# ronen-halevy/yolo-v3-tf2

Hardware: AMD Instinct MI355X
Metric: images/sec at 416x416 batch=64, f32 (full YOLOv3 detect: conv stack + decode + NMS) (higher is better)
Workload: dtype f32

## Files before the change

### include/y3.h

```cpp
#ifndef Y3_H
#define Y3_H

#include <stddef.h>
#include <stdint.h>

#ifdef __cplusplus
extern "C" {
#endif

typedef int y3_status;
enum {
    Y3_OK = 0,
    Y3_ERR_INVALID = -1,
    Y3_ERR_HIP = -2,
    Y3_ERR_OOM = -3,
    Y3_ERR_STATE = -4,
    Y3_ERR_NODEVICE = -5,
    Y3_ERR_COMM = -6,
    Y3_ERR_INTERNAL = -7
};

enum { Y3_DTYPE_F32 = 0, Y3_DTYPE_BF16 = 1, Y3_DTYPE_F32X3 = 2, Y3_DTYPE_F32X2 = 3, Y3_DTYPE_F16 = 4, Y3_DTYPE_I8 = 5 };

int y3_version(void);
// ... 37 lines not shown
                        const y3_conv_desc *convs, int n_convs, const y3_aux_desc *aux, int n_aux,
                        int input_tensor, const int32_t outputs[3], int nclasses, y3_net **out);
void y3_net_destroy(y3_net *net);

y3_status y3_net_set_conv_weights(y3_net *net, int conv_slot, const float *w, const float *gamma,
                                  const float *beta, const float *mean, const float *var, const float *bias,
                                  float eps);

y3_status y3_net_set_tile(y3_net *net, int conv_slot, int tile);
y3_status y3_net_set_tile_bf16(y3_net *net, int conv_slot, int tile);
y3_status y3_net_set_tile_x3(y3_net *net, int conv_slot, int tile);
y3_status y3_net_set_tile_x2(y3_net *net, int conv_slot, int tile);
y3_status y3_net_set_lanes(y3_net *net, int lanes);
y3_status y3_net_set_xcd_mode(y3_net *net, int mode);
y3_status y3_net_set_k_chunk(y3_net *net, int channels);
y3_status y3_net_set_low_latency(y3_net *net, int on);
y3_status y3_net_set_split_k(y3_net *net, int conv_slot, int S);
int y3_net_get_split_k(const y3_net *net, int conv_slot);
int y3_choose_split_k(long long tiles, int k_tiles, int n_cus, long long slab_bytes_per_slice);
y3_status y3_net_set_low_latency_bf16(y3_net *net, int on);
y3_status y3_net_set_split_k_bf16(y3_net *net, int conv_slot, int S);
int y3_net_get_split_k_bf16(const y3_net *net, int conv_slot);
y3_status y3_net_set_low_latency_f16(y3_net *net, int on);
y3_status y3_net_set_split_k_f16(y3_net *net, int conv_slot, int S);
int y3_net_get_split_k_f16(const y3_net *net, int conv_slot);
y3_status y3_net_keep_activations(y3_net *net, int keep);
y3_status y3_net_set_stem_fusion(y3_net *net, int on);
y3_status y3_net_set_stem_fusion_f16(y3_net *net, int on);
y3_status y3_net_measure_sclk(y3_net *net, const float *images_dev, int batch, float *const grids_dev[3], int forwards,
                              float *mhz_out, void *stream);
// ... 107 lines not shown
```

### yolo-v3-tf2_amd/_lib.py

```python
from __future__ import annotations

import ctypes as C
import os

from . import PACKAGE_DIR

LIB_PATH = os.environ.get("Y3_LIB_PATH") or os.path.join(PACKAGE_DIR, "lib", "liby3hip.so")

Y3_OK = 0
Y3_DTYPE_F32, Y3_DTYPE_BF16, Y3_DTYPE_F32X3, Y3_DTYPE_F32X2, Y3_DTYPE_F16, Y3_DTYPE_I8 = 0, 1, 2, 3, 4, 5
DTYPE_TAGS = {Y3_DTYPE_F32: "f32", Y3_DTYPE_BF16: "bf16", Y3_DTYPE_F32X3: "f32x3", Y3_DTYPE_F32X2: "f32x2", Y3_DTYPE_F16: "f16", Y3_DTYPE_I8: "i8"}
TILES_I8_BUILT = (8, 10, 11, 12, 17, 19, 24, 26, 27, 29)
TILES_X2_BUILT = (0, 1, 2, 3, 4, 8, 12, 26, 27)
TILES_X3_BUILT = (0, 1, 2, 3, 4, 8, 9, 12, 13, 14)
Y3_AUX_ADD, Y3_AUX_UPSAMPLE2X, Y3_AUX_CONCAT = 0, 1, 2
_Z = (0, 0, 0, 0)
TILES = [_Z, _Z, _Z, _Z, _Z, _Z,
         (128, 128, 4, 1), _Z, (256, 32, 4, 1), (128, 64, 4, 1), (64, 128, 4, 1), (64, 64, 4, 1),
         (128, 128, 8, 1), _Z, _Z, _Z,
         _Z, (128, 64, 8, 1), _Z, _Z,
         _Z, _Z, _Z,
         (128, 128, 4, 1), _Z,
         _Z,
         (64, 128, 4, 2), (64, 64, 4, 2), _Z, _Z, _Z,
# ... 57 lines not shown
    "y3_device_count": (_i, []),
    "y3_tile_built": (_i, [_i, _i]),
    "y3_net_create": (_i, [C.POINTER(TensorDesc), _i, C.POINTER(C.c_int32), _i, C.POINTER(ConvDesc), _i,
                           C.POINTER(AuxDesc), _i, _i, C.POINTER(C.c_int32), _i, C.POINTER(_vp)]),
    "y3_net_destroy": (None, [_vp]),
    "y3_net_set_conv_weights": (_i, [_vp, _i, _fp, _fp, _fp, _fp, _fp, _fp, _f]),
    "y3_net_set_tile": (_i, [_vp, _i, _i]),
    "y3_net_set_tile_bf16": (_i, [_vp, _i, _i]),
    "y3_net_set_tile_x3": (_i, [_vp, _i, _i]),
    "y3_net_set_tile_x2": (_i, [_vp, _i, _i]),
    "y3_net_set_early_chunk": (_i, [_vp, _i, _i]),
    "y3_net_keep_activations": (_i, [_vp, _i]),
    "y3_net_set_lanes": (_i, [_vp, _i]),
    "y3_net_set_xcd_mode": (_i, [_vp, _i]),
    "y3_net_set_k_chunk": (_i, [_vp, _i]),
    "y3_net_set_stem_fusion": (_i, [_vp, _i]),
    "y3_net_set_low_latency": (_i, [_vp, _i]),
    "y3_net_set_split_k": (_i, [_vp, _i, _i]),
    "y3_net_get_split_k": (_i, [_vp, _i]),
    "y3_choose_split_k": (_i, [C.c_longlong, _i, _i, C.c_longlong]),
    "y3_net_set_low_latency_bf16": (_i, [_vp, _i]),
    "y3_net_set_split_k_bf16": (_i, [_vp, _i, _i]),
    "y3_net_get_split_k_bf16": (_i, [_vp, _i]),
    "y3_net_set_low_latency_f16": (_i, [_vp, _i]),
    "y3_net_set_split_k_f16": (_i, [_vp, _i, _i]),
    "y3_net_get_split_k_f16": (_i, [_vp, _i]),
    "y3_net_set_stem_fusion_f16": (_i, [_vp, _i]),
    "y3_net_measure_sclk": (_i, [_vp, _vp, _i, C.POINTER(_vp), _i, _fp, _vp]),
    "y3_net_measure_sclk_conv": (_i, [_vp, _vp, _i, C.POINTER(_vp), _i, _i, _fp, _vp]),
    "y3_net_measure_sclk_all": (_i, [_vp, _vp, _i, C.POINTER(_vp), _i, _fp, C.POINTER(C.c_double), C.POINTER(C.c_double), _vp]),
# ... 92 lines not shown
```

### yolo-v3-tf2_amd/csrc/conv_common.h

```cpp
#pragma once
#include "y3_device.h"
#include "y3_kernels.h"

namespace y3 {

struct TileOrigin { int b0, ho0, wo0; float rcpW, rcpH; };

__device__ __forceinline__ TileOrigin tile_origin(const ConvArgs &p, int m0)
{
    TileOrigin t;
    const int HoWo = p.Ho * p.Wo;
    t.b0 = m0 / HoWo;
    const int r0 = m0 - t.b0 * HoWo;
    t.ho0 = r0 / p.Wo;
    t.wo0 = r0 - t.ho0 * p.Wo;
    t.rcpW = 1.0f / (float)p.Wo;
    t.rcpH = 1.0f / (float)p.Ho;
    return t;
}

__device__ __forceinline__ void tile_row(const ConvArgs &p, const TileOrigin &t, int x, int &b, int &ho, int &wo)
{
    const int qx = (int)(((float)x + 0.5f) * t.rcpW);
    wo = x - qx * p.Wo;
// ... 9 lines not shown
    int b, ho, wo;
    tile_row(p, t, x, b, ho, wo);
    if (CONCAT) {
        const int H0 = p.up0 ? (p.H >> 1) : p.H, W0 = p.up0 ? (p.W >> 1) : p.W;
        const int h0 = p.up0 ? (ho >> 1) : ho, w0 = p.up0 ? (wo >> 1) : wo;
        aoff = ((b * H0 + h0) * W0 + w0) * EPC * p.C0;
        aoff1 = ((b * p.H + ho) * p.W + wo) * EPC * c1;
        ahw = (m < p.M) ? 0 : (int)0x80000000;
    } else {
        const int hi0 = ho * p.stride - p.pad, wi0 = wo * p.stride - p.pad;
        aoff = ((b * p.H + hi0) * p.W + wi0) * EPC * p.Cin;
        ahw = (m < p.M) ? ((hi0 << 16) | (wi0 & 0xffff)) : (int)0x80000000;
    }
}

template <int LPR>
__device__ __forceinline__ int swizzled_chunk(int row, int chunk)
{
    static_assert(LPR == 2 || LPR == 4 || LPR == 8, "16-byte chunks per LDS row");
    constexpr int SHIFT = (LPR == 8) ? 1 : (LPR == 4) ? 2 : 3;
    return chunk ^ ((row >> SHIFT) & (LPR - 1));
}

__device__ __forceinline__ constexpr int mfma32_row(int e, int fh = 0) { return 4 * fh + (e & 3) + 8 * (e >> 2); }
__device__ __forceinline__ constexpr int mfma16_row(int e, int fh, int mb = 0) { return 16 * mb + 4 * fh + e; }

}
```

### yolo-v3-tf2_amd/csrc/conv_f32.hip

```cpp
#include <algorithm>
#include <type_traits>

#include "conv_common.h"

namespace y3 {

static constexpr int BK = 32;
static constexpr int lds_row(int dma) { return dma ? BK : BK + 4; }

__device__ __forceinline__ f32x4 buf_load16(__amdgpu_buffer_rsrc_t r, unsigned voff, int soff)
{
    u32x4 v = __builtin_amdgcn_raw_buffer_load_b128(r, (int)voff, soff, 0);
    return __builtin_bit_cast(f32x4, v);
}

#ifdef Y3_PHASE_STAMPS
__device__ unsigned long long y3_dbg32_stamps[8 * 32768];
__device__ int y3_dbg32_sel_k = -1;
#define Y3_STAMP32(k) do { if (threadIdx.x == 0 && blockIdx.x < 32768 && p.K == y3_dbg32_sel_k) y3_dbg32_stamps[blockIdx.x * 8 + (k)] = __builtin_amdgcn_s_memrealtime(); } while (0)
#else
#define Y3_STAMP32(k) do { } while (0)
#endif

template <int TM, int TN, int WR, int WC, bool CONCAT, int STAGES, int MINW = 1, int DMA = 0, bool SPLIT = false>
__global__ __launch_bounds__(64 * WR * WC, MINW) void conv_f32_mfma(const ConvArgs p)
{
    static_assert(!SPLIT || (!DMA && STAGES == 1), "the split-K form is built for the register-staged single-stage tiles");
    Y3_STAMP32(0);
#ifdef Y3_PHASE_STAMPS
    if (threadIdx.x == 0 && blockIdx.x < 32768 && p.K == y3_dbg32_sel_k) {
        y3_dbg32_stamps[blockIdx.x * 8 + 5] = __builtin_amdgcn_s_getreg((31 << 11) | 4);
        y3_dbg32_stamps[blockIdx.x * 8 + 6] = __builtin_amdgcn_s_getreg((31 << 11) | 20);
    }
#endif
    static_assert(DMA || STAGES == 1, "register-staged operand loads are single-stage; two stages need the LDS-DMA loads");
    constexpr int LDS_ROW = lds_row(DMA);
    constexpr int BM = 32 * TM * WR;
    constexpr int BN = 32 * TN * WC;
    constexpr int NT = 64 * WR * WC;
    constexpr int RP = NT / 8;
    constexpr int AP = BM / RP;
    constexpr int BP = BN / RP;
    static_assert(BM % RP == 0 && BN % RP == 0 && AP >= 1 && BP >= 1, "tile too small for the thread count");
    constexpr int STAGE = (BM + BN) * LDS_ROW;
    extern __shared__ __attribute__((aligned(16))) float smem[];

    const int tid = threadIdx.x;
    if constexpr (!SPLIT) clk_stamp_entry(p.clk_stamps);
    const int lane = tid & 63;
    const int wave = __builtin_amdgcn_readfirstlane(tid >> 6);
    const int wr = wave / WC, wc = wave % WC;

    const int nwg = gridDim.x;
    const int bid = blockIdx.x, xcd = bid & 7;
    const int logical = xcd_contiguous_tile(bid, nwg);
    const int tilesN = p.CoutPad / BN;
    const int kt0 = SPLIT ? (int)blockIdx.y * (p.K / BK) / (int)gridDim.y : 0;
    const int KT = SPLIT ? ((int)blockIdx.y + 1) * (p.K / BK) / (int)gridDim.y - kt0 : p.K / BK;
    const __amdgpu_buffer_rsrc_t rs0 = buffer_rsrc(p.src0, p.src0_bytes);
    const __amdgpu_buffer_rsrc_t rs1 = buffer_rsrc(CONCAT ? p.src1 : p.src0, CONCAT ? p.src1_bytes : p.src0_bytes);
    const __amdgpu_buffer_rsrc_t rsw = buffer_rsrc(p.wpk, p.w_bytes);
    const unsigned OOB0 = p.src0_bytes, OOB1 = CONCAT ? p.src1_bytes : p.src0_bytes;

    const __amdgpu_buffer_rsrc_t rsd = buffer_rsrc(p.dst, p.dst_bytes);
    const __amdgpu_buffer_rsrc_t rsr = buffer_rsrc(p.residual ? p.residual : p.dst, p.dst_bytes);
    const int fr = lane & 31, fh = lane >> 5;

    int mt = logical / tilesN, nt = logical - mt * tilesN;
    if (p.xcd_gn > 0) {
        const int gn = p.xcd_gn, gm = 8 / gn;
        const int tilesM = (p.M + BM - 1) / BM;
        const int xm = xcd / gn, xn = xcd - xm * gn;
        const int nb = tilesN / gn;
        const int mlo = xm * tilesM / gm, mhi = (xm + 1) * tilesM / gm;
        const int j = bid >> 3;
        const int lm = j / nb;
        mt = mlo + lm;
        nt = xn * nb + (j - lm * nb);
        if (mt >= mhi) return;
    }
    const int m0 = mt * BM, n0 = nt * BN;

    const int lrow = tid >> 3;
    const int lchunk = DMA ? swizzled_chunk<8>(lrow, tid & 7) * 4 : (tid & 7) * 4;
    int aoff[AP];
    int aoff1[CONCAT ? AP : 1];
    int ahw[AP];
    const int C1 = p.Cin - p.C0;
    const TileOrigin org = tile_origin(p, m0);
#pragma unroll
    for (int i = 0; i < AP; ++i)
        gather_row<CONCAT, 1>(p, org, m0 + i * RP + lrow, org.wo0 + i * RP + lrow, C1, aoff[i], aoff1[CONCAT ? i : 0], ahw[i]);
    unsigned boff[BP];
#pragma unroll
    for (int j = 0; j < BP; ++j) boff[j] = (unsigned)((n0 + j * RP + lrow) * p.K + lchunk) * 4u;

    const int CK = (!CONCAT && p.k_chunk > 0 && p.k_chunk < p.Cin) ? p.k_chunk : p.Cin;
    int kglob = 0;
    int tap = 0;
    int c0 = 0;
    int cend = CK;
    const int taps = p.ksize * p.ksize;
    if constexpr (SPLIT) {
        const int tpc = CK / BK, per_chunk = taps * tpc;
        const int chunk = kt0 / per_chunk, r = kt0 - chunk * per_chunk;
        tap = r / tpc;
        c0 = chunk * CK + (r - tap * tpc) * BK;
        cend = (chunk + 1) * CK;
        kglob = tap * p.Cin + c0;
    }
    unsigned avoff[AP];
    unsigned okmask[CONCAT ? 1 : AP];
    unsigned abase4[CONCAT ? 1 : AP];
    unsigned avoff1[CONCAT ? AP : 1];
    auto set_tap = [&]() {
        if (CONCAT) {
#pragma unroll
            for (int i = 0; i < AP; ++i) {
                avoff[i] = (ahw[i] < 0) ? OOB0 : (unsigned)(aoff[i] + lchunk) * 4u;
                avoff1[i] = (ahw[i] < 0) ? OOB1 : (unsigned)(aoff1[i] + lchunk) * 4u;
            }
        } else {
            const int u = tap / p.ksize, v = tap - u * p.ksize;
            const unsigned toff4 = (unsigned)((u * p.W + v) * p.Cin) * 4u;
#pragma unroll
            for (int i = 0; i < AP; ++i) avoff[i] = ((okmask[i] >> tap) & 1u) ? abase4[i] + toff4 : OOB0;
        }
    };
    if (!CONCAT) {
#pragma unroll
        for (int i = 0; i < AP; ++i) {
            unsigned mk = 0;
            if (ahw[i] >= 0 || (ahw[i] >> 16) != -32768) {
                const int hi0 = ahw[i] >> 16, wi0 = (int)(short)(ahw[i] & 0xffff);
                if (p.ksize == 3) {
                    const unsigned H = (unsigned)p.H, W = (unsigned)p.W;
                    const unsigned rm = ((unsigned)hi0 < H ? 7u : 0u) | ((unsigned)(hi0 + 1) < H ? 56u : 0u) | ((unsigned)(hi0 + 2) < H ? 448u : 0u);
                    const unsigned cm = ((unsigned)wi0 < W ? 1u : 0u) | ((unsigned)(wi0 + 1) < W ? 2u : 0u) | ((unsigned)(wi0 + 2) < W ? 4u : 0u);
                    mk = rm & (cm * 73u);
                } else {
                    for (int u = 0; u < p.ksize; ++u)
                        for (int v = 0; v < p.ksize; ++v)
                            if ((unsigned)(hi0 + u) < (unsigned)p.H && (unsigned)(wi0 + v) < (unsigned)p.W) mk |= 1u << (u * p.ksize + v);
                }
            }
            okmask[i] = mk;
            abase4[i] = (unsigned)(aoff[i] + lchunk) * 4u;
        }
    }
    set_tap();

    auto advance_k = [&]() {
        c0 += BK;
        if (c0 == cend) {
            ++tap;
            if (!CONCAT && tap == taps && cend != p.Cin) {
                tap = 0;
                cend += CK;
            }
            c0 = cend - CK;
            if (!CONCAT) set_tap();
        }
        kglob = tap * p.Cin + c0;
    };

    f32x4 ra[AP], rb[BP];
    auto fetch_dma = [&](int buf) {
        float *sa = smem + buf * STAGE + wave * 8 * LDS_ROW;
        float *sb = sa + BM * LDS_ROW;
        if (CONCAT && c0 >= p.C0) {
#pragma unroll
            for (int i = 0; i < AP; ++i)
// ... 48 lines not shown
        asm volatile("s_waitcnt vmcnt(0)" ::: "memory");
    } else {
        fetch();
        stage(0);
    }
    __syncthreads();
    Y3_STAMP32(2);

    const int a_frag = (wr * 32 * TM + fr) * LDS_ROW + (DMA ? 0 : fh * 4);
    const int b_frag = BM * LDS_ROW + (wc * 32 * TN + fr) * LDS_ROW + (DMA ? 0 : fh * 4);
    int foff[4];
#pragma unroll
    for (int q = 0; q < 4; ++q) foff[q] = DMA ? swizzled_chunk<8>(fr, 2 * q + fh) * 4 : q * 8;

    const bool interior = (m0 + BM <= p.M) && (n0 + BN <= p.Cout);
    const int row_bytes = p.Cout * 4;

    for (int kt = 0; kt < KT; ++kt) {
        const int cur = (STAGES == 2) ? (kt & 1) : 0;
        if (DMA && STAGES == 2) {
            if (kt + 1 < KT) fetch_dma(cur ^ 1);
        } else if (!DMA) {
            if (kt + 1 < KT) fetch();
        }
        const float *sa = smem + cur * STAGE + a_frag;
        const float *sb = smem + cur * STAGE + b_frag;
#pragma unroll
        for (int q = 0; q < 4; ++q) {
            f32x4 fa[TM], fb[TN];
#pragma unroll
            for (int i = 0; i < TM; ++i) fa[i] = *reinterpret_cast<const f32x4 *>(sa + i * 32 * LDS_ROW + foff[q]);
// ... 41 lines not shown
                                                          mfma32_row(e) * slab_row_bytes, 0);
            }
        }
    } else {
    auto emit = [&](auto leaky_tag, auto res_tag, auto interior_tag) {
        constexpr bool LEAKY = decltype(leaky_tag)::value, RES = decltype(res_tag)::value;
        constexpr bool interior = decltype(interior_tag)::value;
#pragma unroll
        for (int j = 0; j < TN; ++j) {
            const int n = n0 + (wc * TN + j) * 32 + fr;
            const float sh = p.shift[n];
            const bool n_ok = n < p.Cout;
#pragma unroll
            for (int i = 0; i < TM; ++i) {
                const int mbase = m0 + (wr * TM + i) * 32 + 4 * fh;
                const unsigned vbase = (unsigned)(mbase * p.Cout + n) * 4u;
                unsigned off[16];
                if (!interior) {
#pragma unroll
                    for (int e = 0; e < 16; ++e) {
                        const int m = mbase + mfma32_row(e);
                        off[e] = (n_ok && m < p.M) ? (unsigned)(m * p.Cout + n) * 4u : p.dst_bytes;
                    }
                }
                float r[16];
                if (RES) {
#pragma unroll
                    for (int e = 0; e < 16; ++e) {
                        const int so = mfma32_row(e) * row_bytes;
                        r[e] = __builtin_bit_cast(float, interior ? __builtin_amdgcn_raw_buffer_load_b32(rsr, (int)vbase, so, 0)
                                                                  : __builtin_amdgcn_raw_buffer_load_b32(rsr, (int)off[e], 0, 0));
                    }
                }
#pragma unroll
                for (int e = 0; e < 16; e += 2) {
                    f32x2 v2 = f32x2{acc[i][j][e], acc[i][j][e + 1]} + f32x2{sh, sh};
                    if (LEAKY) {
// ... 56 lines not shown
}

template <int TM, int TN, int WR, int WC, bool CONCAT, int STAGES, int MINW, int DMA>
static hipError_t launch_k(const ConvArgs &a, hipStream_t s)
{
    constexpr int BM = 32 * TM * WR, BN = 32 * TN * WC;
    const int tilesM = (a.M + BM - 1) / BM, tilesN = a.CoutPad / BN;
    const size_t lds = STAGES * (size_t)(BM + BN) * lds_row(DMA) * sizeof(float);
    int grid = tilesM * tilesN;
    if (a.xcd_gn > 0) {
        if (8 % a.xcd_gn || tilesN % a.xcd_gn) return hipErrorInvalidValue;
        const int gm = 8 / a.xcd_gn;
        int rows = 0;
        for (int xm = 0; xm < gm; ++xm) rows = std::max(rows, (xm + 1) * tilesM / gm - xm * tilesM / gm);
        grid = 8 * rows * (tilesN / a.xcd_gn);
    }
    return launch_conv_kernel<conv_f32_mfma<TM, TN, WR, WC, CONCAT, STAGES, MINW, DMA>>(a, grid, 64 * WR * WC, lds, s);
}

template <int TM, int TN, int WR, int WC, int STAGES, int MINW, int DMA>
static hipError_t launch_t(const ConvArgs &a, hipStream_t s)
{
    return a.src1 ? launch_k<TM, TN, WR, WC, true, STAGES, MINW, DMA>(a, s) : launch_k<TM, TN, WR, WC, false, STAGES, MINW, DMA>(a, s);
}

struct TileF32 { TileInfo info; hipError_t (*launch)(const ConvArgs &, hipStream_t); };
template <int TM, int TN, int WR, int WC, int STAGES = 1, int MINW = 1, int DMA = 0>
static constexpr TileF32 tile() { return {{32 * TM * WR, 32 * TN * WC, WR * WC, STAGES, BK}, launch_t<TM, TN, WR, WC, STAGES, MINW, DMA>}; }

static hipError_t launch_res(const ConvArgs &a, hipStream_t s) { return conv_res_f32_fits(a) ? launch_conv_res_f32(a, s) : hipErrorInvalidValue; }
// ... 71 lines not shown
```

### yolo-v3-tf2_amd/csrc/y3_forward.cpp

```cpp
#include <cstdlib>
#include <vector>

#include "y3_host.h"

struct Forward {
    const float *images;
    float *const *grids;
    int batch;
    hipStream_t stream;
    int lanes;
    const y3::DecodeHead *heads = nullptr;
    unsigned long long *clk = nullptr;
    int clk_conv = -1;
    float *ms_out = nullptr;
    int n_ms = 0;
};

static y3_status check_forward_args(const y3_net *net, bool args_ok, int batch, bool heads, const char *who)
{
    if (!net || !args_ok || batch <= 0) return fail(Y3_ERR_INVALID, "%s: bad argument", who);
    if (heads && net->nclasses <= 0) return fail(Y3_ERR_STATE, "%s: the net was created without detection heads (nclasses = 0)", who);
    if (!net->height) return fail(Y3_ERR_STATE, "%s: call y3_net_plan first", who);
    if (batch > net->max_batch) return fail(Y3_ERR_INVALID, "%s: batch %d > planned %d", who, batch, net->max_batch);
    return Y3_OK;
// ... 176 lines not shown
            HIP_TRY(hipEventCreate(&ev1));
        }
        if (op_begin == 0 && crosses(net->input_tensor))
            if (y3_status st = quantize_crossing(net->input_tensor); st != Y3_OK) return st;
        for (int oi = op_begin; oi < op_end; ++oi) {
            const Op &o = net->ops[oi];
            if (o.kind != 0) {
                if (y3_status st = run_aux(o.index); st != Y3_OK) return st;
                continue;
            }
            y3::ConvArgs a = conv_args(o.index);
            if (!a.src0 || (!a.dst && !a.dec.boxes)) return fail(Y3_ERR_STATE, "conv %d: tensor not planned", o.index);
            const y3::ConvChoice ch = y3::choose_conv(net, oi, a);
            a.k_chunk = ch.k_chunk;
            a.xcd_gn = ch.xcd_gn;
            if (ch.kind == y3::ConvKind::InStem) {
                if (f.ms_out && o.index < f.n_ms) f.ms_out[o.index] = 0.0f;
            } else {
                if (f.ms_out) HIP_TRY(hipEventRecord(ev0, s));
                if (y3_status st = launch_conv(oi, a, ch); st != Y3_OK) return st;
                if (f.ms_out) {
                    HIP_TRY(hipEventRecord(ev1, s));
                    HIP_TRY(hipEventSynchronize(ev1));
                    float ms = 0;
                    HIP_TRY(hipEventElapsedTime(&ms, ev0, ev1));
                    if (o.index < f.n_ms) f.ms_out[o.index] = ms;
                }
            }
            const int dst = net->convs[o.index].d.dst;
            if (crosses(dst))
// ... 338 lines not shown
```

### yolo-v3-tf2_amd/csrc/y3_host.h

```cpp
#pragma once
#include <hip/hip_runtime.h>

#include <vector>

#include "../../include/y3.h"
#include "y3_kernels.h"

namespace y3 {
int fail_msg(int code, const char *fmt, ...) noexcept;
int on_exception(const char *who) noexcept;
bool test_fail_alloc() noexcept;
}

#define Y3_CATCH(who) catch (...) { return y3::on_exception(who); }

constexpr auto fail = y3::fail_msg;

#define HIP_TRY(expr)                                                                             \
    do {                                                                                          \
        hipError_t e_ = (expr);                                                                   \
        if (e_ != hipSuccess)                                                                     \
            return fail(e_ == hipErrorOutOfMemory ? Y3_ERR_OOM : Y3_ERR_HIP, "%s: %s", #expr,     \
                        hipGetErrorString(e_));                                                   \
    } while (0)
// ... 33 lines not shown
    bool x2_ok = true;
    void *wx2_dev = nullptr;
    void *w_dev = nullptr;
    float *w0stem_dev = nullptr;
    float *w0raw_dev = nullptr;
    float *w0norm_dev = nullptr;
    float *scale0norm_dev = nullptr;
    void *wbf_dev = nullptr;
    void *wf16_dev = nullptr;
    float *scale_dev = nullptr;
    float *shift_dev = nullptr;
    void *wi8_dev = nullptr;
    std::vector<float> sw_host, bn_scale_host;
    float *sc_i8_dev = nullptr;
    float q_res = 0.0f, q_inv = 0.0f;
};

struct Op {
    int kind;
    int index;
};

constexpr int Y3_MAX_LANES = 4;
constexpr int Y3_MAX_OUTPUT_BOXES = 1024;

struct y3_net {
    int device = 0;
    int n_cus = 0;
    std::vector<y3_tensor_desc> tensors;
    std::vector<Op> ops;
// ... 15 lines not shown
    size_t det_bytes = 0;
    int stem_mode = 1;
    bool stem_mode_set = false;
    int stem_mode_f16 = 0;
    bool stem_fused = false;
    bool stem_conv2 = false;
    int xcd_mode = 1;
    bool low_latency_set = false;
    bool low_latency = false;
    bool low_latency_bf16 = false;
    bool low_latency_f16 = false;
    void *split_ws = nullptr;
    size_t split_ws_lane = 0;
    int split_ws_lanes = 0;
    int k_chunk = -1;
    hipEvent_t fork_ev = nullptr;
    hipStream_t lane_stream[4] = {nullptr, nullptr, nullptr, nullptr};
    hipEvent_t join_ev[4] = {nullptr, nullptr, nullptr, nullptr};
    std::vector<void *> tdev;
    std::vector<size_t> tbytes;
    std::vector<size_t> tblock;
    std::vector<void *> blocks;
    std::vector<float> act_scale;
    int i8_first_conv = -1;
    std::vector<unsigned char> telem;
    std::vector<char> tcross;
    std::vector<void *> tq8;
    std::vector<float> tscale;
};

// ... 37 lines not shown
    const SplitForm *split;
};
const ConvFamily *conv_family(int dtype);
inline const ConvFamily &family_of(const y3_net *net) { return *conv_family(net->dtype); }
inline bool conv_is_i8(const y3_net *net, int slot) { return net->dtype == Y3_DTYPE_I8 && net->i8_first_conv >= 0 && slot >= net->i8_first_conv; }
inline int dtype_of_conv(const y3_net *net, int slot) { return net->dtype != Y3_DTYPE_I8 || conv_is_i8(net, slot) ? net->dtype : (int)Y3_DTYPE_F16; }
inline const ConvFamily &family_of_conv(const y3_net *net, int slot) { return *conv_family(dtype_of_conv(net, slot)); }

enum class ConvKind { First, Stem, InStem, HeadDecodeF32, Mfma, SplitK };
struct ConvChoice {
    ConvKind kind;
    int tile;
    int k_chunk;
    int xcd_gn;
    int split_k;
};
ConvChoice choose_conv(const y3_net *net, int oi, const ConvArgs &a);
ConvChoice choose_conv_planned(const y3_net *net, int oi);
int conv_op(const y3_net *net, int slot);

bool stem_applicable(const y3_net *net);
bool stem_conv2_applicable(const y3_net *net);
void resolve_stem(y3_net *net);
bool output_staged(const y3_net *net, int t);
y3_status resolve_splits(y3_net *net);
y3_status resolve_i8(y3_net *net);
y3_status upload_i8_scales(y3_net *net, int slot);
void free_plan(y3_net *net);

struct DetectLayout {
    int32_t gs[3][2];
    size_t n_boxes;
    size_t grid[3], boxes, cls, scores, sel, nms_ws, total;
};
DetectLayout detect_layout(const y3_net *net, int batch);

y3_status decode_scores_hw(const char *who, const float *const grids_dev[3], const int32_t (*grid_hw)[2], int batch, int nclasses,
                           const float *anchors_host, float *bboxes_dev, int64_t *class_idx_dev, float *scores_dev, void *stream);

}
// ... 1 lines not shown
```

### yolo-v3-tf2_amd/csrc/y3_kernels.h

```cpp
#pragma once
#include <hip/hip_runtime.h>
#include <stddef.h>
#include <stdint.h>
#include <type_traits>

#include "../../include/y3.h"
#include "decode_box.h"

namespace y3 {

struct ConvArgs {
    const void *src0;
    const void *src1;
    const void *wpk;
    const float *scale;
    const float *shift;
    const void *residual;
    void *dst;
    int B, H, W;
    int Ho, Wo;
    int Cin, C0;
    int Cout, CoutPad;
    int ksize, stride, pad;
    int up0;
    int leaky;
    int M;
    int K;
    unsigned src0_bytes, src1_bytes, w_bytes, dst_bytes;
    int xcd_gn;
    DecodeHead dec;
    int k_chunk;
    unsigned long long *clk_stamps;
    int n_cus;
    int device;
    float q_res, q_inv;
};

struct LdsAttrOnce { unsigned long long done = 0; };
inline hipError_t set_max_lds_once(LdsAttrOnce &st, const void *fn, int bytes, int dev = -1)
{
    hipError_t e = hipSuccess;
    if (dev < 0 && (e = hipGetDevice(&dev)) != hipSuccess) return e;
    if (dev >= 0 && dev < 64 && ((st.done >> dev) & 1ull)) return hipSuccess;
    e = hipFuncSetAttribute(fn, hipFuncAttributeMaxDynamicSharedMemorySize, bytes);
    if (e == hipSuccess && dev >= 0 && dev < 64) st.done |= 1ull << dev;
    return e;
}

template <auto KERNEL>
static hipError_t launch_conv_kernel(const ConvArgs &a, int grid, int threads, size_t lds, hipStream_t s, int grid_y = 1)
{
// ... 162 lines not shown
```

### yolo-v3-tf2_amd/csrc/y3_net.cpp

```cpp
#include <algorithm>
#include <cmath>
#include <cstdarg>
#include <cstdio>
#include <cstdlib>
#include <cstring>
#include <exception>
#include <memory>
#include <new>

#include "y3_host.h"

namespace {

thread_local char g_err[512] = "";

}

namespace y3 {
int fail_msg(int code, const char *fmt, ...) noexcept
{
    va_list ap;
    va_start(ap, fmt);
    vsnprintf(g_err, sizeof(g_err), fmt, ap);
    va_end(ap);
// ... 199 lines not shown
}

int choose_tile_i8(const ConvSlot &c, long long M, long long M_plan, bool arena_out)
{
    const int t = choose_tile_bf16(c, M, M_plan, arena_out);
    if (y3::conv_i8_tile_built(t) && fits(y3::conv_i8_tile_info(t), c, c.cout_pad64)) return t;
    static constexpr int n64[] = {10, 11};
    return first_reaching(n64, y3::conv_i8_tile_info, c, c.cout_pad64, M, 512);
}

int default_k_chunk(const ConvSlot &c)
{
    static const int env = [] { const char *e = getenv("Y3_K_CHUNK"); return e ? atoi(e) : -1; }();
    if (env >= 0) return env;
    return (c.d.size == 3 && c.d.cin >= 256) ? 128 : 0;
}

int choose_xcd_gn(const ConvSlot &c, const y3::ConvArgs &a, const y3::TileInfo &t)
{
    const int tilesN = a.CoutPad / t.bn;
    const long long tilesM = (a.M + t.bm - 1) / t.bm;
    if (tilesM * tilesN < 64) return 0;
    const double w_bytes = (double)a.CoutPad * c.K * 4.0, a_bytes = (double)a.src0_bytes + a.src1_bytes;
    int best = 0;
    double best_cost = 0;
    for (int gn = 1; gn <= 8; gn *= 2) {
        const int gm = 8 / gn;
        if (tilesN % gn || tilesM < gm) continue;
        double cost = gn * a_bytes + gm * w_bytes;
        if (w_bytes / gn > 2.5e6) cost += 8.0 * (a_bytes + w_bytes);
// ... 80 lines not shown
    if (!(c.d.size == 3 && c.d.stride == 1 && c.d.src1 < 0 && (c.d.cin == 32 || c.d.cin == 64) && c.d.cout % 64 == 0))
        return fail(Y3_ERR_INVALID, "y3_net_set_tile_bf16: tile 32 (weight-resident) needs a 3x3 / stride-1 conv with 32 or 64 input channels and Cout %% 64 == 0");
    if (is_output(net, c.d.dst) && !y3::output_staged(net, c.d.dst))
        return fail(Y3_ERR_INVALID, "y3_net_set_tile_bf16: tile 32 (weight-resident) stores bf16 only; conv %d writes an fp32 net output", slot);
    return Y3_OK;
}

void refine_f32(const y3_net *net, const ConvSlot &c, const y3::ConvArgs &a, y3::ConvChoice &ch)
{
    if (a.dec.boxes) { ch.kind = y3::ConvKind::HeadDecodeF32; return; }
    ch.split_k = c.split_k;
    if (c.split_k > 1) ch.kind = y3::ConvKind::SplitK;
    else if (net->xcd_mode) ch.xcd_gn = choose_xcd_gn(c, a, y3::conv_tile_info(ch.tile));
    const int ck = net->k_chunk >= 0 ? net->k_chunk : default_k_chunk(c);
    if (c.d.size == 3 && c.d.src1 < 0 && ck > 0 && c.d.cin > ck && c.d.cin % ck == 0 && ck % 32 == 0) ch.k_chunk = ck;
}

void refine_bf16(const y3_net *, const ConvSlot &c, const y3::ConvArgs &a, y3::ConvChoice &ch)
{
    if (c.split_k > 1 && !a.dec.boxes) {
        ch.split_k = c.split_k;
        ch.kind = y3::ConvKind::SplitK;
        return;
    }
    if (a.dec.boxes && y3::conv_bf16_tile_info(ch.tile).bn != 256) {
        const bool m16 = ch.tile >= 24 && ch.tile <= 29;
        const bool big = (a.M + 255) / 256 >= 256;
        ch.tile = m16 ? (big ? 24 : 26) : (big ? 17 : 19);
    }
}
// ... 421 lines not shown
}
Y3_CATCH("y3_net_set_stem_fusion")

y3_status y3_net_set_stem_fusion_f16(y3_net *net, int on)
try { return set_stem_fusion("y3_net_set_stem_fusion_f16", net, &y3_net::stem_mode_f16, on); }
Y3_CATCH("y3_net_set_stem_fusion_f16")

y3_status y3_net_set_k_chunk(y3_net *net, int channels)
try {
    if (!net || channels < -1 || (channels > 0 && channels % 32)) return fail(Y3_ERR_INVALID, "y3_net_set_k_chunk: -1, 0 or a multiple of 32 channels");
    net->k_chunk = channels;
    return Y3_OK;
}
Y3_CATCH("y3_net_set_k_chunk")

y3_status y3_net_set_low_latency(y3_net *net, int on)
try { return set_low_latency(F32_FAMILY, net, on, &y3_net::low_latency_set); }
Y3_CATCH("y3_net_set_low_latency")

y3_status y3_net_set_split_k(y3_net *net, int slot, int S)
try { return set_split_k(F32_FAMILY, net, slot, S); }
Y3_CATCH("y3_net_set_split_k")

y3_status y3_net_set_low_latency_bf16(y3_net *net, int on)
try { return set_low_latency(BF16_FAMILY, net, on); }
Y3_CATCH("y3_net_set_low_latency_bf16")

y3_status y3_net_set_split_k_bf16(y3_net *net, int slot, int S)
try { return set_split_k(BF16_FAMILY, net, slot, S); }
Y3_CATCH("y3_net_set_split_k_bf16")
// ... 77 lines not shown
```

### yolo-v3-tf2_amd/csrc/y3_plan.cpp

```cpp
#include <algorithm>
#include <cstdlib>

#include "y3_host.h"

void y3::free_plan(y3_net *n)
{
    if (n->det_buf) (void)hipFree(n->det_buf);
    n->det_buf = nullptr;
    n->det_bytes = 0;
    if (n->split_ws) (void)hipFree(n->split_ws);
    n->split_ws = nullptr;
    n->split_ws_lane = 0;
    n->split_ws_lanes = 0;
    for (void *p : n->blocks) (void)hipFree(p);
    n->blocks.clear();
    n->tdev.assign(n->tensors.size(), nullptr);
    n->tq8.assign(n->tensors.size(), nullptr);
}

static y3_status ensure_lanes(y3_net *net)
{
    if (net->fork_ev) return Y3_OK;
    HIP_TRY(hipEventCreateWithFlags(&net->fork_ev, hipEventDisableTiming));
    for (int i = 0; i < Y3_MAX_LANES; ++i) {
        HIP_TRY(hipStreamCreateWithFlags(&net->lane_stream[i], hipStreamNonBlocking));
        HIP_TRY(hipEventCreateWithFlags(&net->join_ev[i], hipEventDisableTiming));
    }
    return Y3_OK;
}

static y3_status place_tensors(y3_net *net, const std::vector<int> &first, const std::vector<int> &last)
{
// ... 221 lines not shown
        if ((env == 0 || env == 1) && !net->low_latency_set) net->low_latency = env == 1;
    }
    if (net->nclasses > 0) {
        const size_t bytes = y3::detect_layout(net, max_batch).total;
        hipError_t e = hipMalloc(&net->det_buf, bytes);
        if (e != hipSuccess) {
            y3::free_plan(net);
            return fail(Y3_ERR_OOM, "y3_net_plan: hipMalloc(%zu) for the detect scratch failed: %s", bytes, hipGetErrorString(e));
        }
        net->det_bytes = bytes;
    }
    if (y3_status st = y3::resolve_splits(net); st != Y3_OK) {
        y3::free_plan(net);
        return st;
    }
    return Y3_OK;
}
Y3_CATCH("y3_net_plan_hw")

y3_status y3_net_plan(y3_net *net, int max_batch, int image_size, int dtype)
try {
    return y3_net_plan_hw(net, max_batch, image_size, image_size, dtype);
}
Y3_CATCH("y3_net_plan")

double y3_net_flops_per_image(const y3_net *net)
{
    if (!net || !net->height) return 0.0;
    double tot = 0;
    for (const ConvSlot &c : net->convs) {
        const double ho = net->height / c.d.out_div, wo = net->width / c.d.out_div;
        tot += 2.0 * c.d.size * c.d.size * c.d.cin * c.d.cout * ho * wo;
    }
// ... 5 lines not shown
```

### yolo-v3-tf2_amd/runtime.py

```python
from __future__ import annotations

import ctypes as C
from typing import Dict, List, Optional, Sequence

import numpy as np
import torch

from . import _lib
from ._lib import AuxDesc, ConvDesc, TensorDesc, Y3Error, check
from .graph import AuxOp, ConvOp, Program
from .weights import BN_EPS

_AUX_KIND = {"add": _lib.Y3_AUX_ADD, "upsample": _lib.Y3_AUX_UPSAMPLE2X, "concat": _lib.Y3_AUX_CONCAT}


def _fptr(a: Optional[np.ndarray]):
    if a is None:
        return None
    return a.ctypes.data_as(C.POINTER(C.c_float))


def _dev(t: Optional[torch.Tensor]):
    return C.c_void_p(t.data_ptr()) if t is not None else None

# ... 115 lines not shown
            check(st, f"y3_net_set_conv_weights(conv{i})")
        self.weights_loaded = True

    def keep_activations(self, keep=True):
        check(self.lib.y3_net_keep_activations(self._h, int(keep)), "y3_net_keep_activations")

    def set_lanes(self, lanes: int):
        check(self.lib.y3_net_set_lanes(self._h, int(lanes)), "y3_net_set_lanes")
        self.lanes = int(lanes)

    def set_xcd_mode(self, mode: int):
        check(self.lib.y3_net_set_xcd_mode(self._h, int(mode)), "y3_net_set_xcd_mode")

    def set_k_chunk(self, channels: int):
        check(self.lib.y3_net_set_k_chunk(self._h, int(channels)), "y3_net_set_k_chunk")

    @staticmethod
    def _dtype_arg(dtype) -> int:
        if dtype is None:
            return _lib.Y3_DTYPE_F32
        if isinstance(dtype, str) and dtype in _lib.DTYPE_TAGS.values():
            return next(k for k, v in _lib.DTYPE_TAGS.items() if v == dtype)
        if not isinstance(dtype, (bool, np.bool_)) and isinstance(dtype, (int, np.integer)) and int(dtype) in _lib.DTYPE_TAGS:
            return int(dtype)
        raise Y3Error(f"dtype must be None or one of {sorted(_lib.DTYPE_TAGS.values())} (got {dtype!r})")

    def set_dtype(self, dtype):
        dtype = self._dtype_arg(dtype)
        if self.max_batch and dtype != self.dtype:
            self.plan(self.max_batch, self.image_size, dtype)
# ... 902 lines not shown
```

Before: 2051.

## Reorder 3x3 conv rows by border mask to skip padded taps

Adds a batch-minor row ordering for 3x3 f32 MFMA convs. Output positions are sorted by their valid-tap mask through a device position table, and each 32-image block shares one position, so a tile only iterates the union of live taps and skips zero-padding taps at borders. The output scatter uses a strided batch-minor address, and the K loop length is computed per tile. It is enabled by default wherever legal (batch a multiple of 32), at the cost of scattered output stores and changed memory access patterns for interior tiles.

```diff
diff --git a/include/y3.h b/include/y3.h
--- a/include/y3.h
+++ b/include/y3.h
@@ -75,6 +75,9 @@
 y3_status y3_net_set_lanes(y3_net *net, int lanes);
 y3_status y3_net_set_xcd_mode(y3_net *net, int mode);
 y3_status y3_net_set_k_chunk(y3_net *net, int channels);
+y3_status y3_net_set_border_skip(y3_net *net, int mode);
+int y3_net_get_border_skip(const y3_net *net, int conv_slot, int batch);
+void y3_border_order(int Ho, int Wo, int H, int W, int stride, int pad, uint32_t *out);
 y3_status y3_net_set_low_latency(y3_net *net, int on);
 y3_status y3_net_set_split_k(y3_net *net, int conv_slot, int S);
 int y3_net_get_split_k(const y3_net *net, int conv_slot);
diff --git a/yolo-v3-tf2_amd/_lib.py b/yolo-v3-tf2_amd/_lib.py
--- a/yolo-v3-tf2_amd/_lib.py
+++ b/yolo-v3-tf2_amd/_lib.py
@@ -95,6 +95,9 @@
     "y3_net_set_lanes": (_i, [_vp, _i]),
     "y3_net_set_xcd_mode": (_i, [_vp, _i]),
     "y3_net_set_k_chunk": (_i, [_vp, _i]),
+    "y3_net_set_border_skip": (_i, [_vp, _i]),
+    "y3_net_get_border_skip": (_i, [_vp, _i, _i]),
+    "y3_border_order": (None, [_i, _i, _i, _i, _i, _i, C.POINTER(C.c_uint32)]),
     "y3_net_set_stem_fusion": (_i, [_vp, _i]),
     "y3_net_set_low_latency": (_i, [_vp, _i]),
     "y3_net_set_split_k": (_i, [_vp, _i, _i]),
diff --git a/yolo-v3-tf2_amd/csrc/conv_common.h b/yolo-v3-tf2_amd/csrc/conv_common.h
--- a/yolo-v3-tf2_amd/csrc/conv_common.h
+++ b/yolo-v3-tf2_amd/csrc/conv_common.h
@@ -47,6 +47,49 @@
     }
 }
 
+struct TileBlocks { int j0, r0, n32; unsigned live; };
+
+__device__ __forceinline__ unsigned pos_entry(const ConvArgs &p, int j)
+{
+    const int n = p.Ho * p.Wo;
+    return (unsigned)__builtin_amdgcn_readfirstlane((int)p.pos_tab[j < n ? j : n]);
+}
+
+template <int NBLK>
+__device__ __forceinline__ TileBlocks tile_blocks(const ConvArgs &p, int m0)
+{
+    TileBlocks t;
+    t.n32 = p.B >> 5;
+    const int g0 = m0 >> 5;
+    t.j0 = t.n32 == 1 ? g0 : g0 / t.n32;
+    t.r0 = g0 - t.j0 * t.n32;
+    t.live = 0;
+    int j = t.j0, r = t.r0;
+#pragma unroll
+    for (int k = 0; k < NBLK; ++k) {
+        t.live |= pos_mask(pos_entry(p, j));
+        if (++r == t.n32) {
+            r = 0;
+            ++j;
+        }
+    }
+    return t;
+}
+
+template <int NBLK>
+__device__ __forceinline__ void tile_block(const ConvArgs &p, const TileBlocks &t, int kb, unsigned &ent, int &img)
+{
+    int j = t.j0, r = t.r0 + kb;
+#pragma unroll
+    for (int w = 1; w < NBLK; ++w)
+        if (r >= t.n32) {
+            r -= t.n32;
+            ++j;
+        }
+    ent = pos_entry(p, j);
+    img = r << 5;
+}
+
 template <int LPR>
 __device__ __forceinline__ int swizzled_chunk(int row, int chunk)
 {
diff --git a/yolo-v3-tf2_amd/csrc/conv_f32.hip b/yolo-v3-tf2_amd/csrc/conv_f32.hip
--- a/yolo-v3-tf2_amd/csrc/conv_f32.hip
+++ b/yolo-v3-tf2_amd/csrc/conv_f32.hip
@@ -22,10 +22,11 @@
 #define Y3_STAMP32(k) do { } while (0)
 #endif
 
-template <int TM, int TN, int WR, int WC, bool CONCAT, int STAGES, int MINW = 1, int DMA = 0, bool SPLIT = false>
+template <int TM, int TN, int WR, int WC, bool CONCAT, int STAGES, int MINW = 1, int DMA = 0, bool SPLIT = false, bool BMIN = false>
 __global__ __launch_bounds__(64 * WR * WC, MINW) void conv_f32_mfma(const ConvArgs p)
 {
     static_assert(!SPLIT || (!DMA && STAGES == 1), "the split-K form is built for the register-staged single-stage tiles");
+    static_assert(!BMIN || (!CONCAT && !SPLIT), "batch-minor rows are built for the unsplit single-source launch");
     Y3_STAMP32(0);
 #ifdef Y3_PHASE_STAMPS
     if (threadIdx.x == 0 && blockIdx.x < 32768 && p.K == y3_dbg32_sel_k) {
@@ -56,7 +57,7 @@
     const int logical = xcd_contiguous_tile(bid, nwg);
     const int tilesN = p.CoutPad / BN;
     const int kt0 = SPLIT ? (int)blockIdx.y * (p.K / BK) / (int)gridDim.y : 0;
-    const int KT = SPLIT ? ((int)blockIdx.y + 1) * (p.K / BK) / (int)gridDim.y - kt0 : p.K / BK;
+    int KT = SPLIT ? ((int)blockIdx.y + 1) * (p.K / BK) / (int)gridDim.y - kt0 : p.K / BK;
     const __amdgpu_buffer_rsrc_t rs0 = buffer_rsrc(p.src0, p.src0_bytes);
     const __amdgpu_buffer_rsrc_t rs1 = buffer_rsrc(CONCAT ? p.src1 : p.src0, CONCAT ? p.src1_bytes : p.src0_bytes);
     const __amdgpu_buffer_rsrc_t rsw = buffer_rsrc(p.wpk, p.w_bytes);
@@ -87,17 +88,30 @@
     int aoff1[CONCAT ? AP : 1];
     int ahw[AP];
     const int C1 = p.Cin - p.C0;
-    const TileOrigin org = tile_origin(p, m0);
-#pragma unroll
-    for (int i = 0; i < AP; ++i)
-        gather_row<CONCAT, 1>(p, org, m0 + i * RP + lrow, org.wo0 + i * RP + lrow, C1, aoff[i], aoff1[CONCAT ? i : 0], ahw[i]);
+    constexpr int NBLK = BMIN ? BM / 32 : 1;
+    TileBlocks blk{0, 0, 1, 0x1ffu};
+    unsigned eent[BMIN ? TM : 1];
+    int eimg[BMIN ? TM : 1];
+    if constexpr (BMIN) {
+        blk = tile_blocks<NBLK>(p, m0);
+        if (blk.live == 0) blk.live = 1;
+        KT = __builtin_popcount(blk.live) * (p.Cin / BK);
+#pragma unroll
+        for (int i = 0; i < TM; ++i) tile_block<NBLK>(p, blk, wr * TM + i, eent[i], eimg[i]);
+    } else {
+        const TileOrigin org = tile_origin(p, m0);
+#pragma unroll
+        for (int i = 0; i < AP; ++i)
+            gather_row<CONCAT, 1>(p, org, m0 + i * RP + lrow, org.wo0 + i * RP + lrow, C1, aoff[i], aoff1[CONCAT ? i : 0], ahw[i]);
+    }
+    const int tap0 = BMIN ? __builtin_ctz(blk.live) : 0;
     unsigned boff[BP];
 #pragma unroll
     for (int j = 0; j < BP; ++j) boff[j] = (unsigned)((n0 + j * RP + lrow) * p.K + lchunk) * 4u;
 
     const int CK = (!CONCAT && p.k_chunk > 0 && p.k_chunk < p.Cin) ? p.k_chunk : p.Cin;
-    int kglob = 0;
-    int tap = 0;
+    int tap = tap0;
+    int kglob = BMIN ? tap * p.Cin : 0;
     int c0 = 0;
     int cend = CK;
     const int taps = p.ksize * p.ksize;
@@ -127,7 +141,20 @@
             for (int i = 0; i < AP; ++i) avoff[i] = ((okmask[i] >> tap) & 1u) ? abase4[i] + toff4 : OOB0;
         }
     };
-    if (!CONCAT) {
+    if constexpr (BMIN) {
+        static_assert(RP == 32 || RP == 64, "a load pass covers one or two 32-row blocks");
+#pragma unroll
+        for (int i = 0; i < AP; ++i) {
+            unsigned e;
+            int b;
+            tile_block<NBLK>(p, blk, RP == 32 ? i : 2 * i + (wave >> 2), e, b);
+            b += lrow & 31;
+            const int hi0 = pos_ho(e) * p.stride - p.pad, wi0 = pos_wo(e) * p.stride - p.pad;
+            aoff[i] = ((b * p.H + hi0) * p.W + wi0) * p.Cin;
+            okmask[i] = pos_mask(e);
+            abase4[i] = (unsigned)(aoff[i] + lchunk) * 4u;
+        }
+    } else if (!CONCAT) {
 #pragma unroll
         for (int i = 0; i < AP; ++i) {
             unsigned mk = 0;
@@ -153,9 +180,14 @@
     auto advance_k = [&]() {
         c0 += BK;
         if (c0 == cend) {
-            ++tap;
+            if constexpr (BMIN) {
+                const unsigned rest = blk.live >> (tap + 1);
+                tap = rest ? tap + 1 + __builtin_ctz(rest) : taps;
+            } else {
+                ++tap;
+            }
             if (!CONCAT && tap == taps && cend != p.Cin) {
-                tap = 0;
+                tap = tap0;
                 cend += CK;
             }
             c0 = cend - CK;
@@ -234,7 +266,7 @@
     for (int q = 0; q < 4; ++q) foff[q] = DMA ? swizzled_chunk<8>(fr, 2 * q + fh) * 4 : q * 8;
 
     const bool interior = (m0 + BM <= p.M) && (n0 + BN <= p.Cout);
-    const int row_bytes = p.Cout * 4;
+    const int row_bytes = BMIN ? p.Ho * p.Wo * p.Cout * 4 : p.Cout * 4;
 
     for (int kt = 0; kt < KT; ++kt) {
         const int cur = (STAGES == 2) ? (kt & 1) : 0;
@@ -306,13 +338,21 @@
 #pragma unroll
             for (int i = 0; i < TM; ++i) {
                 const int mbase = m0 + (wr * TM + i) * 32 + 4 * fh;
-                const unsigned vbase = (unsigned)(mbase * p.Cout + n) * 4u;
+                unsigned vbase;
+                if constexpr (BMIN) {
+                    const unsigned pe = eent[i];
+                    const int b = eimg[i] + 4 * fh;
+                    vbase = (unsigned)(((b * p.Ho + pos_ho(pe)) * p.Wo + pos_wo(pe)) * p.Cout + n) * 4u;
+                } else {
+                    vbase = (unsigned)(mbase * p.Cout + n) * 4u;
+                }
                 unsigned off[16];
                 if (!interior) {
 #pragma unroll
                     for (int e = 0; e < 16; ++e) {
                         const int m = mbase + mfma32_row(e);
-                        off[e] = (n_ok && m < p.M) ? (unsigned)(m * p.Cout + n) * 4u : p.dst_bytes;
+                        if constexpr (BMIN) off[e] = (n_ok && m < p.M) ? vbase + (unsigned)(mfma32_row(e) * row_bytes) : p.dst_bytes;
+                        else off[e] = (n_ok && m < p.M) ? (unsigned)(m * p.Cout + n) * 4u : p.dst_bytes;
                     }
                 }
                 float r[16];
@@ -399,6 +439,14 @@
         int rows = 0;
         for (int xm = 0; xm < gm; ++xm) rows = std::max(rows, (xm + 1) * tilesM / gm - xm * tilesM / gm);
         grid = 8 * rows * (tilesN / a.xcd_gn);
+    }
+    if constexpr (!CONCAT) {
+        if (a.pos_tab) {
+            if (a.ksize != 3 || a.B < 32 || a.B % 32 || a.M != a.B * a.Ho * a.Wo || a.Ho > kPosMaxGrid || a.Wo > kPosMaxGrid) return hipErrorInvalidValue;
+            return launch_conv_kernel<conv_f32_mfma<TM, TN, WR, WC, false, STAGES, MINW, DMA, false, true>>(a, grid, 64 * WR * WC, lds, s);
+        }
+    } else if (a.pos_tab) {
+        return hipErrorInvalidValue;
     }
     return launch_conv_kernel<conv_f32_mfma<TM, TN, WR, WC, CONCAT, STAGES, MINW, DMA>>(a, grid, 64 * WR * WC, lds, s);
 }
diff --git a/yolo-v3-tf2_amd/csrc/y3_forward.cpp b/yolo-v3-tf2_amd/csrc/y3_forward.cpp
--- a/yolo-v3-tf2_amd/csrc/y3_forward.cpp
+++ b/yolo-v3-tf2_amd/csrc/y3_forward.cpp
@@ -214,6 +214,7 @@
             const y3::ConvChoice ch = y3::choose_conv(net, oi, a);
             a.k_chunk = ch.k_chunk;
             a.xcd_gn = ch.xcd_gn;
+            a.pos_tab = ch.pos_tab;
             if (ch.kind == y3::ConvKind::InStem) {
                 if (f.ms_out && o.index < f.n_ms) f.ms_out[o.index] = 0.0f;
             } else {
diff --git a/yolo-v3-tf2_amd/csrc/y3_host.h b/yolo-v3-tf2_amd/csrc/y3_host.h
--- a/yolo-v3-tf2_amd/csrc/y3_host.h
+++ b/yolo-v3-tf2_amd/csrc/y3_host.h
@@ -71,6 +71,7 @@
     std::vector<float> sw_host, bn_scale_host;
     float *sc_i8_dev = nullptr;
     float q_res = 0.0f, q_inv = 0.0f;
+    const uint32_t *pos_tab = nullptr;
 };
 
 struct Op {
@@ -116,6 +117,9 @@
     size_t split_ws_lane = 0;
     int split_ws_lanes = 0;
     int k_chunk = -1;
+    int border_skip = -1;
+    struct PosTab { int Ho, Wo, H, W, stride; uint32_t *dev; };
+    std::vector<PosTab> pos_tabs;
     hipEvent_t fork_ev = nullptr;
     hipStream_t lane_stream[4] = {nullptr, nullptr, nullptr, nullptr};
     hipEvent_t join_ev[4] = {nullptr, nullptr, nullptr, nullptr};
@@ -183,6 +187,7 @@
     int k_chunk;
     int xcd_gn;
     int split_k;
+    const uint32_t *pos_tab;
 };
 ConvChoice choose_conv(const y3_net *net, int oi, const ConvArgs &a);
 ConvChoice choose_conv_planned(const y3_net *net, int oi);
@@ -193,6 +198,7 @@
 void resolve_stem(y3_net *net);
 bool output_staged(const y3_net *net, int t);
 y3_status resolve_splits(y3_net *net);
+y3_status resolve_border(y3_net *net);
 y3_status resolve_i8(y3_net *net);
 y3_status upload_i8_scales(y3_net *net, int slot);
 void free_plan(y3_net *net);
diff --git a/yolo-v3-tf2_amd/csrc/y3_kernels.h b/yolo-v3-tf2_amd/csrc/y3_kernels.h
--- a/yolo-v3-tf2_amd/csrc/y3_kernels.h
+++ b/yolo-v3-tf2_amd/csrc/y3_kernels.h
@@ -34,7 +34,16 @@
     int n_cus;
     int device;
     float q_res, q_inv;
+    const uint32_t *pos_tab;
 };
+
+constexpr int kPosMaxGrid = 2047;
+constexpr int kPosTabPad = 8;
+constexpr uint32_t pos_pack(int ho, int wo, uint32_t mask9) { return ((uint32_t)ho << 20) | ((uint32_t)wo << 9) | mask9; }
+constexpr int pos_ho(uint32_t e) { return (int)(e >> 20); }
+constexpr int pos_wo(uint32_t e) { return (int)((e >> 9) & 0x7ffu); }
+constexpr uint32_t pos_mask(uint32_t e) { return e & 0x1ffu; }
+void border_order(int Ho, int Wo, int H, int W, int stride, int pad, uint32_t *out);
 
 struct LdsAttrOnce { unsigned long long done = 0; };
 inline hipError_t set_max_lds_once(LdsAttrOnce &st, const void *fn, int bytes, int dev = -1)
diff --git a/yolo-v3-tf2_amd/csrc/y3_net.cpp b/yolo-v3-tf2_amd/csrc/y3_net.cpp
--- a/yolo-v3-tf2_amd/csrc/y3_net.cpp
+++ b/yolo-v3-tf2_amd/csrc/y3_net.cpp
@@ -237,6 +237,14 @@
     static const int env = [] { const char *e = getenv("Y3_K_CHUNK"); return e ? atoi(e) : -1; }();
     if (env >= 0) return env;
     return (c.d.size == 3 && c.d.cin >= 256) ? 128 : 0;
+}
+
+constexpr int kBorderSkipMaxPositions = 1 << 30;
+bool default_border_skip(const y3::ConvArgs &a)
+{
+    static const int env = [] { const char *e = getenv("Y3_BORDER_SKIP"); return e ? atoi(e) : -1; }();
+    static const int max_pos = [] { const char *e = getenv("Y3_BORDER_SKIP_MAX_POS"); return e ? atoi(e) : kBorderSkipMaxPositions; }();
+    return env != 0 && a.Ho * a.Wo <= max_pos;
 }
 
 int choose_xcd_gn(const ConvSlot &c, const y3::ConvArgs &a, const y3::TileInfo &t)
@@ -347,6 +355,9 @@
     else if (net->xcd_mode) ch.xcd_gn = choose_xcd_gn(c, a, y3::conv_tile_info(ch.tile));
     const int ck = net->k_chunk >= 0 ? net->k_chunk : default_k_chunk(c);
     if (c.d.size == 3 && c.d.src1 < 0 && ck > 0 && c.d.cin > ck && c.d.cin % ck == 0 && ck % 32 == 0) ch.k_chunk = ck;
+    const bool legal = c.pos_tab && ch.kind == y3::ConvKind::Mfma && ch.tile != 33 && a.B >= 32 && a.B % 32 == 0 &&
+                       (long long)a.Ho * a.Wo * a.Cout * 4 * 32 < 0x7fffffffLL;
+    if (legal && (net->border_skip >= 0 ? net->border_skip == 1 : default_border_skip(a))) ch.pos_tab = c.pos_tab;
 }
 
 void refine_bf16(const y3_net *, const ConvSlot &c, const y3::ConvArgs &a, y3::ConvChoice &ch)
@@ -798,6 +809,38 @@
 }
 Y3_CATCH("y3_net_set_k_chunk")
 
+y3_status y3_net_set_border_skip(y3_net *net, int mode)
+try {
+    if (!net || mode < -1 || mode > 1) return fail(Y3_ERR_INVALID, "y3_net_set_border_skip: -1 (the rule), 0 (off) or 1 (on wherever legal)");
+    net->border_skip = mode;
+    return Y3_OK;
+}
+Y3_CATCH("y3_net_set_border_skip")
+
+int y3_net_get_border_skip(const y3_net *net, int slot, int batch)
+{
+    if (!net || !net->height || slot < 0 || slot >= (int)net->convs.size() || batch <= 0 || batch > net->max_batch) return 0;
+    const int oi = y3::conv_op(net, slot);
+    if (oi < 0) return 0;
+    const ConvSlot &c = net->convs[slot];
+    int lanes = net->lanes, n = 0;
+    while (lanes > 1 && batch / lanes < 1) --lanes;
+    for (int l = 0; l < lanes; ++l) {
+        int nb = (int)((long long)batch * (l + 1) / lanes) - (int)((long long)batch * l / lanes);
+        if (oi < net->early_ops && nb > net->early_chunk) nb = net->early_chunk;
+        if (nb <= 0) continue;
+        y3::ConvArgs a{};
+        a.B = nb;
+        a.Ho = net->height / c.d.out_div;
+        a.Wo = net->width / c.d.out_div;
+        a.M = nb * a.Ho * a.Wo;
+        a.Cout = c.d.cout;
+        a.CoutPad = c.*y3::family_of_conv(net, slot).cout_pad;
+        n += y3::choose_conv(net, oi, a).pos_tab != nullptr;
+    }
+    return n;
+}
+
 y3_status y3_net_set_low_latency(y3_net *net, int on)
 try { return set_low_latency(F32_FAMILY, net, on, &y3_net::low_latency_set); }
 Y3_CATCH("y3_net_set_low_latency")
diff --git a/yolo-v3-tf2_amd/csrc/y3_plan.cpp b/yolo-v3-tf2_amd/csrc/y3_plan.cpp
--- a/yolo-v3-tf2_amd/csrc/y3_plan.cpp
+++ b/yolo-v3-tf2_amd/csrc/y3_plan.cpp
@@ -12,10 +12,59 @@
     n->split_ws = nullptr;
     n->split_ws_lane = 0;
     n->split_ws_lanes = 0;
+    for (const y3_net::PosTab &t : n->pos_tabs) (void)hipFree(t.dev);
+    n->pos_tabs.clear();
+    for (ConvSlot &c : n->convs) c.pos_tab = nullptr;
     for (void *p : n->blocks) (void)hipFree(p);
     n->blocks.clear();
     n->tdev.assign(n->tensors.size(), nullptr);
     n->tq8.assign(n->tensors.size(), nullptr);
+}
+
+void y3::border_order(int Ho, int Wo, int H, int W, int stride, int pad, uint32_t *out)
+{
+    auto mask_of = [&](int ho, int wo) {
+        uint32_t mk = 0;
+        for (int u = 0; u < 3; ++u)
+            for (int v = 0; v < 3; ++v) {
+                const int hi = ho * stride - pad + u, wi = wo * stride - pad + v;
+                if (hi >= 0 && hi < H && wi >= 0 && wi < W) mk |= 1u << (u * 3 + v);
+            }
+        return mk;
+    };
+    auto key_of = [](uint32_t mk) { return (uint32_t)__builtin_popcount(mk) * 512u + mk; };
+    std::vector<int> at(10 * 512 + 1, 0);
+    for (int ho = 0; ho < Ho; ++ho)
+        for (int wo = 0; wo < Wo; ++wo) ++at[key_of(mask_of(ho, wo)) + 1];
+    for (int k = 0; k < 10 * 512; ++k) at[k + 1] += at[k];
+    for (int ho = 0; ho < Ho; ++ho)
+        for (int wo = 0; wo < Wo; ++wo) {
+            const uint32_t mk = mask_of(ho, wo);
+            out[at[key_of(mk)]++] = pos_pack(ho, wo, mk);
+        }
+}
+
+y3_status y3::resolve_border(y3_net *net)
+{
+    if (net->dtype != Y3_DTYPE_F32) return Y3_OK;
+    for (ConvSlot &c : net->convs) {
+        const y3_conv_desc &d = c.d;
+        if (d.size != 3 || d.src1 >= 0 || c.first_layer) continue;
+        const y3_net::PosTab g{net->height / d.out_div, net->width / d.out_div, net->height / d.in_div, net->width / d.in_div, d.stride, nullptr};
+        if (g.Ho > kPosMaxGrid || g.Wo > kPosMaxGrid) continue;
+        for (const y3_net::PosTab &t : net->pos_tabs)
+            if (t.Ho == g.Ho && t.Wo == g.Wo && t.H == g.H && t.W == g.W && t.stride == g.stride) c.pos_tab = t.dev;
+        if (c.pos_tab) continue;
+        const size_t n = (size_t)g.Ho * g.Wo;
+        std::vector<uint32_t> tab(n + kPosTabPad, 0u);
+        border_order(g.Ho, g.Wo, g.H, g.W, g.stride, 1, tab.data());
+        net->pos_tabs.push_back(g);
+        y3_net::PosTab &t = net->pos_tabs.back();
+        HIP_TRY(hipMalloc(reinterpret_cast<void **>(&t.dev), tab.size() * sizeof(uint32_t)));
+        HIP_TRY(hipMemcpy(t.dev, tab.data(), tab.size() * sizeof(uint32_t), hipMemcpyHostToDevice));
+        c.pos_tab = t.dev;
+    }
+    return Y3_OK;
 }
 
 static y3_status ensure_lanes(y3_net *net)
@@ -267,9 +316,18 @@
         y3::free_plan(net);
         return st;
     }
+    if (y3_status st = y3::resolve_border(net); st != Y3_OK) {
+        y3::free_plan(net);
+        return st;
+    }
     return Y3_OK;
 }
 Y3_CATCH("y3_net_plan_hw")
+
+void y3_border_order(int Ho, int Wo, int H, int W, int stride, int pad, uint32_t *out)
+{
+    if (out && Ho > 0 && Wo > 0 && Ho <= y3::kPosMaxGrid && Wo <= y3::kPosMaxGrid) y3::border_order(Ho, Wo, H, W, stride, pad, out);
+}
 
 y3_status y3_net_plan(y3_net *net, int max_batch, int image_size, int dtype)
 try {
diff --git a/yolo-v3-tf2_amd/runtime.py b/yolo-v3-tf2_amd/runtime.py
--- a/yolo-v3-tf2_amd/runtime.py
+++ b/yolo-v3-tf2_amd/runtime.py
@@ -153,6 +153,12 @@
 
     def set_k_chunk(self, channels: int):
         check(self.lib.y3_net_set_k_chunk(self._h, int(channels)), "y3_net_set_k_chunk")
+
+    def set_border_skip(self, mode: int):
+        check(self.lib.y3_net_set_border_skip(self._h, int(mode)), "y3_net_set_border_skip")
+
+    def border_skip(self, slot: int, batch: int) -> int:
+        return int(self.lib.y3_net_get_border_skip(self._h, int(slot), int(batch)))
 
     @staticmethod
     def _dtype_arg(dtype) -> int:
```

Result: faster. 2093 (median of 6 runs) (+2.0%).
